# sloisel/MultiGridBarrier.jl

Hardware: AMD Instinct MI355X
Metric: Newton iters/sec + wall-clock to converge, 2D P2 p-Laplace L=9 (higher is better)
Workload: dtype f64

## Files before the change

include/mgbhip.h:

```cpp
#ifndef MGBHIP_H
#define MGBHIP_H

#include <stdint.h>

#ifdef __cplusplus
extern "C" {
#endif

#define MGBHIP_OK 0
#define MGBHIP_ERR_INVALID 1
#define MGBHIP_ERR_HIP 2
#define MGBHIP_ERR_NOT_SPD 3
#define MGBHIP_ERR_NONFINITE 4
#define MGBHIP_ERR_CONVERGENCE 5

#define MGBHIP_MAX_PIECES 4
#define MGBHIP_MAX_IDX 10
#define MGBHIP_MAX_LIN 4
#define MGBHIP_MAX_ND 13
#define MGBHIP_MAX_NU 4
#define MGBHIP_MAX_OPS 8

#define MGBHIP_KIND_EP 1
#define MGBHIP_KIND_LINEAR 2
// ... 139 lines not shown
                const mgbhip_vec* z0, mgbhip_vec* grad);
int mgbhip_f2_d(mgbhip_problem* prob, int32_t level, const mgbhip_vec* s, const mgbhip_vec* c,
                const mgbhip_vec* z0);
int mgbhip_solve_d(mgbhip_problem* prob, int32_t level, const mgbhip_vec* g, mgbhip_vec* x);
int mgbhip_prolong_add(mgbhip_problem* prob, int32_t level, const mgbhip_vec* s, mgbhip_vec* z);

int mgbhip_stage_ms(mgbhip_problem* prob, const char* stage, double* total_ms, int64_t* launches);
int mgbhip_reset_stage_timers(mgbhip_problem* prob, int enable);
int mgbhip_solver_stats(mgbhip_problem* prob, int32_t level, double* out8);
int mgbhip_solver_chain(mgbhip_problem* prob, int32_t level, double* out8);
enum { MGBHIP_PROJ_NONE = 0, MGBHIP_PROJ_LOOP = 1, MGBHIP_PROJ_STAGED = 2, MGBHIP_PROJ_MFMA = 3, MGBHIP_PROJ_ACCUMULATE = 4 };
int mgbhip_level_plan(mgbhip_problem* prob, int32_t level, int32_t* out16);
enum { MGBHIP_ELEM_F0 = 0, MGBHIP_ELEM_F1 = 1, MGBHIP_ELEM_F2 = 2, MGBHIP_ELEM_NODE_F = 3, MGBHIP_ELEM_NODE_SLACK = 4, MGBHIP_ELEM_F01 = 5 };
enum { MGBHIP_ELEM_KIND_DENSE = 0, MGBHIP_ELEM_KIND_WIDE = 1, MGBHIP_ELEM_KIND_FAST_DEFAULT = 2, MGBHIP_ELEM_KIND_FAST_RUNTIME = 3,
       MGBHIP_ELEM_KIND_CONDENSE = 4, MGBHIP_ELEM_KIND_GENERIC = 5 };
int mgbhip_elem_plan(mgbhip_problem* prob, int32_t mode, int32_t* out16);
int mgbhip_trial_values(mgbhip_problem* prob, int32_t level, const double* x, const double* dir, double step, const double* c,
                        const double* z0, double* y, double* g, double* xn, int32_t* moved, int32_t* finite, int32_t* path);
enum { MGBHIP_LAUNCH_ROW = 16 };
enum { MGBHIP_ASM_NONE = 0, MGBHIP_ASM_GATHER = 1, MGBHIP_ASM_COLUMNS = 2 };
enum { MGBHIP_B0_NA = 0, MGBHIP_B0_GATHER = 1, MGBHIP_B0_DIAG0 = 2, MGBHIP_B0_STEP0 = 3 };
enum { MGBHIP_BWD_NA = 0, MGBHIP_BWD_K8 = 1, MGBHIP_BWD_K16 = 2, MGBHIP_BWD_GENERAL = 3 };
int64_t mgbhip_solver_launches(mgbhip_problem* prob, int32_t level, int32_t* out, int64_t cap);

#define MGBHIP_INTERP_FEM1D 1
#define MGBHIP_INTERP_QK 2
#define MGBHIP_INTERP_P1 3
#define MGBHIP_INTERP_P2 4
#define MGBHIP_INTERP_SPECTRAL1D 5
#define MGBHIP_INTERP_SPECTRAL2D 6
#define MGBHIP_INTERP_P2C 7
int mgbhip_interpolate(mgbhip_ctx* ctx, int32_t family, int32_t d, int32_t k, int32_t p, int64_t N,
                       const double* x, const double* table, int32_t ncomp, const double* z, int64_t M,
                       const double* pts, double* out, int32_t* elem);
int mgbhip_interpolate_grad(mgbhip_ctx* ctx, int32_t family, int32_t d, int32_t k, int32_t p, int64_t N,
                            const double* x, const double* table, int32_t ncomp, const double* z, int64_t M,
                            const double* pts, double* out ,
                            double* grad , int32_t* elem );

typedef struct mgbhip_locator mgbhip_locator;
int mgbhip_locator_create(mgbhip_ctx* ctx, int32_t family, int32_t d, int32_t k, int32_t p, int64_t N,
                          const double* x, const double* table, int64_t M, const double* pts,
                          mgbhip_locator** out);
int mgbhip_locator_elements(const mgbhip_locator* loc, int32_t* elem );
int mgbhip_locator_evaluate(mgbhip_locator* loc, int32_t ncomp, const double* z ,
                            double* out ,
// ... 148 lines not shown
```

multigridbarrier.jl_amd/csrc/api.cpp:

```cpp
#include <chrono>
#include <cmath>
#include <cstring>
#include <algorithm>
#include <limits>
#include <memory>
#include <string>

#include "closest.hpp"
#include "contour.hpp"
#include "figure.hpp"
#include "interpolate.hpp"
#include "polyline.hpp"
#include "problem.hpp"
#include "quadrature.hpp"
#include "raycast.hpp"
#include "stream.hpp"
#include "surface.hpp"
#include "tubes.hpp"
#include "weld.hpp"

using namespace mgbhip;

mgbhip_problem* problem_create(mgbhip_ctx* ctx, const mgbhip_problem_desc* d, mgbhip_problem* share);
int core_run(mgbhip_problem* P, double* z, const double* c, const mgbhip_options* opt, mgbhip_core_result* res);
// ... 734 lines not shown
int mgbhip_solver_chain(mgbhip_problem* P, int32_t level, double* out) {
    MGB_API_BEGIN
    check_level(P, level);
    MGB_REQUIRE(out != nullptr, "null argument");
    MGB_REQUIRE(P->levels[level].solver.analyzed, "mgbhip_solver_chain: the level has not been factored yet");
    P->levels[level].solver.chain_stats(out);
    return MGBHIP_OK;
    MGB_API_END
}

static_assert(MGBHIP_LAUNCH_ROW == mgbhip::MF_LAUNCH_ROW && MGBHIP_ASM_GATHER == mgbhip::MF_ASM_GATHER &&
              MGBHIP_ASM_COLUMNS == mgbhip::MF_ASM_COLS && MGBHIP_B0_GATHER == mgbhip::MF_B0_GATHER &&
              MGBHIP_B0_DIAG0 == mgbhip::MF_B0_DIAG0 && MGBHIP_B0_STEP0 == mgbhip::MF_B0_STEP0 && MGBHIP_BWD_K8 == mgbhip::MF_BWD_K8 &&
              MGBHIP_BWD_K16 == mgbhip::MF_BWD_K16 && MGBHIP_BWD_GENERAL == mgbhip::MF_BWD_GENERAL, "mgbhip.h and mf_launch_plan.hpp disagree");

int64_t mgbhip_solver_launches(mgbhip_problem* P, int32_t level, int32_t* out, int64_t cap) {
    int64_t count = 0;
    const int rc = [&]() -> int {
        MGB_API_BEGIN
        check_level(P, level);
        MGB_REQUIRE(cap >= 0 && (out != nullptr || cap == 0), "bad output buffer");
        MGB_REQUIRE(P->levels[level].solver.analyzed, "mgbhip_solver_launches: the level has not been factored yet");
        count = P->levels[level].solver.launches(out, cap);
        return MGBHIP_OK;
        MGB_API_END
    }();
    return rc == MGBHIP_OK ? count : -(int64_t)rc;
}

#ifdef MGB_STEP_PROBE
int mgbhip_debug_probe(long long* out64) { (void)hipDeviceSynchronize(); mgbhip::mf_debug_probe(out64); return 0; }
#endif

int mgbhip_reset_stage_timers(mgbhip_problem* P, int enable) {
    MGB_API_BEGIN_ON(P)
    MGB_REQUIRE(P, "null argument");
    P->ctx->timers.reset(enable != 0);
    return MGBHIP_OK;
    MGB_API_END
}

static void interpolate_check_geometry(InterpIn& in) {
    const int32_t family = in.family, d = in.d, k = in.k, p = in.p;
    const int64_t N = in.N;
    const double* x = in.x;
    const bool fem = interp_is_fem(family);
// ... 799 lines not shown
```

multigridbarrier.jl_amd/csrc/mf_launch_plan.hpp:

```cpp
#pragma once
#include <algorithm>
#include <cstdint>
#include <cstdlib>
#include <vector>

#include "host_util.hpp"
#include "mf_analysis.hpp"

namespace mgbhip {

struct MfLaunch {
    int32_t first, count;
    int32_t cls;
    int32_t max_m, max_k;
    int32_t max_child = 0;
    bool tiny = false;
    bool wave = false;
    bool inv = false;
    bool iface = false;
    int32_t grec_first = -1;
};

constexpr int BIG_INV_MAX_M = 7000;
constexpr int GATHER_MAX_CHILD = 8;
constexpr int BIG_DIAG0_MIN_COUNT = 24;

struct MfSwitches {
    bool no_geo;
    bool old_big;
    bool merge_groups;
    bool packed_leaves;
    bool wave_small;
    int64_t inv_min_n;
    int64_t wave_min_n;
    bool gather_lds_maps;
    int gather_ct;
    bool bwd_split;
    static MfSwitches from_env() {
        auto num = [](const char* name, long long dflt) { const char* e = getenv(name); return e ? atoll(e) : dflt; };
        return {env_on("MGBHIP_NO_GEO"), env_on("MGBHIP_OLD_BIG"), !env_on("MGBHIP_NO_MERGE_GROUPS"), !env_on("MGBHIP_NO_PACKED_LEAVES"),
                !env_on("MGBHIP_NO_WAVE_SMALL"), num("MGBHIP_INV_MIN_N", 1024), num("MGBHIP_WAVE_MIN_N", 0),
                env_on("MGBHIP_GATHER_LDS_MAPS"), (int)num("MGBHIP_GATHER_CT", 0), num("MGBHIP_BWD_SPLIT", 1) != 0};
    }
};

using LevelLaunches = std::vector<std::vector<MfLaunch>>;

inline MfLaunch launch_of_range(const MfPlan& plan, MfLaunch L, int32_t first, int32_t count) {
    L.first = first; L.count = count;
    L.max_m = 0; L.max_k = 0; L.max_child = 0;
    for (int32_t t = first; t < first + count; ++t) {
        L.max_m = std::max(L.max_m, plan.fronts[t].m);
        L.max_k = std::max(L.max_k, plan.fronts[t].k);
        L.max_child = std::max(L.max_child, plan.fronts[t].nchild);
    }
    return L;
}

inline void merge_straggler_groups(const MfPlan& plan, std::vector<MfLaunch>& G) {
    auto absorb = [&](size_t into, size_t from) {
        MfLaunch& A = G[into];
        const MfLaunch& B = G[from];
        A.first = B.first;
        A.count += B.count;
        A.max_k = std::max(A.max_k, B.max_k);
// ... 143 lines not shown
    if (forced == 8 || forced == 16 || forced == 32) return forced;
    int ct = 8;
    while (ct < 32 && (int64_t)L.count * ((L.max_m + 2 * ct - 1) / (2 * ct)) >= GATHER_MIN_WGS) ct *= 2;
    return ct;
}

constexpr int BWD_SPLIT_MAX = 16;
constexpr int BWD_SPLIT_CUS = 256;
constexpr int BWD_SPLIT_COLS = 64;
constexpr int BWD_THIN_BOUNDARY = 8;
inline int bwd_inv_split(int32_t count, int32_t max_k, int32_t max_m) {
    if (count < 1 || max_m - max_k <= BWD_THIN_BOUNDARY) return 1;
    return std::max(1, std::min({BWD_SPLIT_MAX, BWD_SPLIT_CUS / count, (max_k + BWD_SPLIT_COLS - 1) / BWD_SPLIT_COLS}));
}
inline int32_t bwd_split_stride(int32_t max_k) { return (max_k + 1) & ~1; }
inline void bwd_split_scratch(const LevelLaunches& solves, int64_t out[2]) {
    out[0] = out[1] = 0;
    for (auto& lev : solves)
        for (auto& L : lev) {
            if (L.count == 0 || L.cls || !L.inv || bwd_inv_split(L.count, L.max_k, L.max_m) == 1) continue;
            out[0] = std::max<int64_t>(out[0], L.count);
            out[1] = std::max<int64_t>(out[1], (int64_t)L.count * bwd_split_stride(L.max_k));
        }
}

struct GatherRec {
    int64_t map_off;
    int64_t base[GATHER_MAX_CHILD];
    int32_t ld[GATHER_MAX_CHILD];
    int32_t bs[GATHER_MAX_CHILD];
};

inline void build_gather_maps(const MfPlan& plan, LevelLaunches& levels, std::vector<GatherRec>& recs, std::vector<int32_t>& gmap) {
    recs.clear();
    gmap.clear();
    for (auto& lev : levels)
        for (auto& L : lev) {
            L.grec_first = -1;
            if (L.count == 0 || big_assembly_kind(L) != MF_ASM_GATHER) continue;
            L.grec_first = (int32_t)recs.size();
            for (int32_t q = L.first; q < L.first + L.count; ++q) {
                const Front& f = plan.fronts[q];
                GatherRec R{};
                R.map_off = (int64_t)gmap.size();
                gmap.resize(gmap.size() + (size_t)f.nchild * (size_t)f.m, -1);
                for (int32_t c = 0; c < f.nchild; ++c) {
// ... 36 lines not shown
```

multigridbarrier.jl_amd/csrc/mf_numeric.hip:

```cpp
#include <hip/hip_runtime.h>

#include <cstdio>

#include <algorithm>
#include <cstdlib>

#include "../../include/mgbhip.h"
#include "mf_solver.hpp"
#include "mf_device.hpp"
#include "mf_small.hpp"
#include "mf_big_subst.hpp"
#include "mf_big_inv.hpp"

namespace mgbhip {

namespace {

int32_t query_lds_cap() {
    if (hipFuncSetAttribute((const void*)mf_factor_small<8, true>, hipFuncAttributeMaxDynamicSharedMemorySize,
                            (int)factor_small_lds(128)) == hipSuccess)
        return 128;
    (void)hipGetLastError();
    return 88;
}
// ... 137 lines not shown

    lds_cap = query_lds_cap();
    const bool inv_ok = !sw.old_big && query_inv_optin();
    level_launches = classify_launches(plan, lds_cap, inv_ok, sw);
    level_solves = merge_level_solves(level_launches);
    uses_inv = false;
    const std::vector<char> on_big_path = fronts_on_big_path(plan, level_launches);
    int32_t max_big = 1;
    for (auto& lev : level_launches)
        for (auto& L : lev) {
            uses_inv = uses_inv || L.inv;
            if (!L.cls) max_big = std::max(max_big, L.count);
        }
    d_dscr.alloc((size_t)max_big * 2 * NB * NB);
    {
        int64_t need[2] = {0, 0};
        if (sw.bwd_split) bwd_split_scratch(level_solves, need);
        if (need[0] == 0) { d_bwd_g.release(); d_bwd_cnt.release(); }
        else {
            d_bwd_g.alloc((size_t)need[1]);
            d_bwd_cnt.alloc((size_t)need[0]);
            d_bwd_cnt.zero(st);
        }
    }

    std::vector<int64_t> ug_ptr, ug_src;
    build_gather_lists(plan, on_big_path, fd, ug_ptr, ug_src);
    leaf_packed = sw.packed_leaves && pack_leaf_fronts(plan, level_launches, on_big_path, fd);
    d_ug_ptr.upload(ug_ptr, st);
    d_ug_src.upload(ug_src, st);
    std::vector<GatherRec> grec;
    std::vector<int32_t> gmap;
    if (!sw.gather_lds_maps) build_gather_maps(plan, level_launches, grec, gmap);
    gather_ct = sw.gather_ct;
    if (grec.empty()) { d_grec.release(); d_gmap.release(); }
    else { d_grec.upload(grec, st); d_gmap.upload(gmap, st); }
    d_fronts.upload(fd, st);
    h_fronts = fd;
    h_a_dst = remap_a_dst(plan, level_launches);
    d_a_dst.upload(h_a_dst, st);
    if (debug_level() >= 2) dump_plan(plan, level_launches);
    analyzed = true;
    MGB_HIP_CHECK(hipStreamSynchronize(st));
}

void MfSolver::set_direct_map(const int32_t* value_map, int64_t nnz, int64_t tail_base, hipStream_t st) {
// ... 86 lines not shown
    if (timers) timers->end();
}

void MfSolver::forward_pass(const double* d_b, hipStream_t st, StageTimers* timers) {
    y_border_one = false;
    y_zero = false;
    const SolveArgs a = solve_args(d_b, nullptr, st);
    int lvno = -1;
    for (auto& lev : level_solves) {
        LevelScope lvscope(timers, "fwd", ++lvno);
        for (auto& L : lev) {
            if (L.count == 0) continue;
            if (L.tiny) launch_forward_tiny(a, L);
            else if (L.cls) launch_forward_small(a, L);
            else if (L.inv && factored_inv) launch_fwd_inv(a, L);
            else if (L.max_m <= BIG1_MAX_M) launch_fwd_big1(a, L);
            else launch_fwd_big_steps(a, L);
        }
    }
}

void MfSolver::backward_pass(double* d_x, hipStream_t st, StageTimers* timers) {
    const SolveArgs a = solve_args(nullptr, d_x, st);
    for (int32_t l = (int32_t)level_solves.size() - 1; l >= 0; --l) {
        LevelScope lvscope(timers, "bwd", l);
        for (auto it = level_solves[l].rbegin(); it != level_solves[l].rend(); ++it) {
            const MfLaunch& L = *it;
            if (L.count == 0) continue;
            if (L.tiny) launch_backward_tiny(a, L);
            else if (L.cls) launch_backward_small(a, L);
            else if (L.inv && factored_inv) launch_bwd_inv(a, L);
            else if (L.max_m <= BIG1_MAX_M) launch_bwd_big1(a, L);
            else launch_bwd_big_steps(a, L);
        }
    }
}

#ifdef MGB_STEP_PROBE
void mf_debug_probe(long long* out64) {
    (void)hipMemcpyFromSymbol(out64, HIP_SYMBOL(g_probe), 64 * sizeof(long long));
    long long init[64];
    for (int i = 0; i < 64; ++i) init[i] = 0;
    init[56] = 0x7fffffffffffffffll;
    (void)hipMemcpyToSymbol(HIP_SYMBOL(g_probe), init, sizeof(init));
}
#endif

void MfSolver::chain_stats(double* out) const {
    double blocks = 0, big_levels = 0, fac = 0, bwd = 0, extra = 0;
    for (auto& lev : level_launches) {
        int lev_blocks = 0;
        for (auto& L : lev) {
            if (L.count == 0) continue;
            if (L.tiny || L.wave || L.cls) { fac += 1; continue; }
            const int nb = (L.max_k + NB - 1) / NB;
            lev_blocks = std::max(lev_blocks, nb);
            fac += 1 + nb + (L.iface ? 3 : 0);
            for (int32_t q = L.first; q < L.first + L.count; ++q) {
                const Front& f = plan.fronts[q];
                const double mk = (double)(f.m - f.k), steps = (double)((f.k + NB - 1) / NB);
                extra += 2.0 * 0.5 * (mk * mk + mk * f.k) * std::max(0.0, steps - 1.0);
            }
        }
        if (lev_blocks) { big_levels += 1; blocks += lev_blocks; }
    }
    for (auto& lev : level_solves)
        for (auto& L : lev)
            if (L.count) bwd += 1;
    out[0] = blocks; out[1] = big_levels; out[2] = fac; out[3] = bwd;
    out[4] = (double)plan.arena_doubles; out[5] = (double)plan.factor_flops; out[6] = extra; out[7] = 0.0;
}

int64_t MfSolver::launches(int32_t* out, int64_t cap) const {
    return launch_rows(level_launches, level_solves, leaf_packed, robust, out, cap);
}

void MfSolver::status_async(int32_t* h_dst2, hipStream_t st) const {
    MGB_HIP_CHECK(hipMemcpyAsync(h_dst2, d_status.p, 2 * sizeof(int32_t), hipMemcpyDeviceToHost, st));
}

int MfSolver::status(hipStream_t st) {
    int32_t h[2] = {0, 0};
    d_status.download(h, 2, st);
    MGB_HIP_CHECK(hipStreamSynchronize(st));
    return status_from(h, factored_condensed);
}

bool MfSolver::enable_condensed(int64_t N, int P, const int32_t* ucol, int64_t slack0, int64_t nnz, int64_t tail_base,
                                hipStream_t st) {
    condensed_ok = false;
    int why = 0;
// ... 70 lines not shown
```

multigridbarrier.jl_amd/csrc/mf_small.hpp:

```cpp
#pragma once
#include "mf_device.hpp"

namespace mgbhip {
namespace {

template <int NBT, bool PACKED>
__global__ void mf_factor_small(const FrontDev* __restrict__ fr, int32_t first,
                                const int32_t* __restrict__ children, const int32_t* __restrict__ rel,
                                const int32_t* __restrict__ a_src, const int32_t* __restrict__ a_dst,
                                const double* __restrict__ Hval, double* __restrict__ arena,
                                int32_t* __restrict__ status) {
    extern __shared__ double W[];
    const FrontDev F = fr[first + blockIdx.x];
    double* Fg = arena + F.F_off;
    const int m = F.m, k = F.k;
    const int tid = threadIdx.x, nt = blockDim.x;
    const int tx = tid % TX, ty = tid / TX, TYn = nt / TX;
    const int mm = PACKED ? m * (m + 1) / 2 : m * m;
    auto co = [m](int c) { return PACKED ? c * (m - 1) - c * (c - 1) / 2 : c * m; };
    double* S = W + mm;

    SP(0);
    int a_d0 = -1;
    double a_v0 = 0.0;
// ... 469 lines not shown
                if (two) s += l1[j] * t1;
                s = wave_sum_f64(s);
                if (lane == j) t0 -= s;
            }
        }
    } else {
        if (lane < m) t0 = (lane < k) ? y[idx[lane]] : x[idx[lane]];
        if (r1 < m) t1 = (r1 < k) ? y[idx[r1]] : x[idx[r1]];
#pragma unroll 2
        for (int j = k - 1; j >= 0; --j) {
            const double* Lj = Fm + (int64_t)j * m;
            double s = 0.0;
            if (lane > j && lane < m) s += Lj[lane] * t0;
            if (r1 > j && r1 < m) s += Lj[r1] * t1;
            s = wave_sum_f64(s);
            if (lane == j) t0 -= s;
            if (r1 == j) t1 -= s;
        }
    }
    if (lane < k) x[idx[lane]] = t0;
    if (r1 < k) x[idx[r1]] = t1;
}

__global__ __launch_bounds__(256) void mf_factor_tiny(const FrontDev* __restrict__ fr, int32_t first, int32_t count,
                                                      const int32_t* __restrict__ a_src,
                                                      const int32_t* __restrict__ a_dst,
                                                      const double* __restrict__ Hval, double* __restrict__ arena,
                                                      int32_t* __restrict__ status) {
    __shared__ double Wt[16][136];
    __shared__ double colb[16][16];
    const int g = threadIdx.x >> 4, r = threadIdx.x & 15;
    const int fi = blockIdx.x * 16 + g;
    const bool on = fi < count;
    const FrontDev F = fr[first + (on ? fi : 0)];
    const int m = F.m, k = on ? F.k : 0;
    double* W = Wt[g];
    for (int i = r; i < 136; i += 16) W[i] = 0.0;
    wave_sync();
    if (on)
        for (int t = r; t < F.a_cnt; t += 16) W[a_dst[F.a_off + t]] = Hval[a_src[F.a_off + t]];
    wave_sync();
    double a[16];
#pragma unroll
    for (int c = 0; c < 16; ++c) a[c] = (on && r < m && c <= r) ? W[c * 16 - c * (c - 1) / 2 + (r - c)] : 0.0;
    int kmax = k;
    kmax = max(kmax, __shfl_xor(kmax, 16, 64));
// ... 117 lines not shown
                       a.values, a.arena, a.status);
}

inline void launch_forward_tiny(const SolveArgs& a, const MfLaunch& L) {
    hipLaunchKernelGGL(mf_forward_tiny, dim3((L.count + 15) / 16), dim3(256), 0, a.st, a.fr, L.first, L.count, a.front_idx,
                       a.arena, a.b, a.y, a.uvec);
}
inline void launch_backward_tiny(const SolveArgs& a, const MfLaunch& L) {
    hipLaunchKernelGGL(mf_backward_tiny, dim3((L.count + 15) / 16), dim3(256), 0, a.st, a.fr, L.first, L.count, a.front_idx,
                       a.arena, a.y, a.x);
}

inline size_t forward_small_lds(int ts) { return (size_t)4 * ts * sizeof(double); }
inline void launch_forward_small(const SolveArgs& a, const MfLaunch& L) {
    const int ts = (L.max_m + 1) & ~1;
    hipLaunchKernelGGL(mf_forward_small, dim3((L.count + 3) / 4), dim3(256), forward_small_lds(ts), a.st, a.fr, L.first, L.count,
                       ts, a.front_idx, a.children, a.rel, a.arena, a.b, a.y, a.uvec);
}
template <int KMAX>
inline void launch_backward_small_k(const SolveArgs& a, const MfLaunch& L) {
    hipLaunchKernelGGL(mf_backward_small<KMAX>, dim3((L.count + 3) / 4), dim3(256), 0, a.st, a.fr, L.first, L.count, a.front_idx,
                       a.arena, a.y, a.x);
}
inline void launch_backward_small(const SolveArgs& a, const MfLaunch& L) {
    const int kmax = backward_small_kmax(L);
    if (kmax == 8) launch_backward_small_k<8>(a, L);
    else if (kmax == 16) launch_backward_small_k<16>(a, L);
    else launch_backward_small_k<0>(a, L);
}

}
}
```

multigridbarrier.jl_amd/csrc/mf_solver.hpp:

```cpp
#pragma once
#include <functional>

#include "common.hpp"
#include "mf_analysis.hpp"
#include "mf_launch_plan.hpp"
#include "kernels.hpp"

namespace mgbhip {

struct FrontDev {
    int32_t k, m, nchild, a_cnt;
    int64_t F_off, idx_off, u_off, child_off, rel_off, a_off, acol_off;
    int64_t ug_off;
    int32_t packed;
    int32_t pad_;
};

struct FactorArgs {
    const FrontDev* fr;
    const int32_t *children, *rel, *a_src, *a_dst, *a_colptr;
    const double* values;
    double *arena, *dscr, *dvec;
    int32_t* status;
    hipStream_t st;
    const GatherRec* grec;
    const int32_t* gmap;
    int gather_ct;
};
struct SolveArgs {
    const FrontDev* fr;
    const int32_t *front_idx, *children, *rel;
    const int64_t *ug_ptr, *ug_src;
    const double *arena, *dvec;
    const double* b;
    double *y, *x, *uvec, *tbig, *tsol;
    hipStream_t st;
    double* bwd_g;
    uint32_t* bwd_cnt;
};

class MfSolver {
   public:
    MfPlan plan;
    void analyze(int64_t n, const int32_t* rowptr, const int32_t* colidx, hipStream_t st,
                 const double* coords = nullptr, int dim = 0, bool protect_peeled = false,
                 const int32_t* top = nullptr, int64_t ntop = 0);
    std::function<void(double*, int64_t)> iface_reduce;
    void factor(const double* d_values, hipStream_t st, StageTimers* timers, bool direct = false, bool condensed = false);
    bool enable_condensed(int64_t N, int P, const int32_t* ucol, int64_t slack0, int64_t nnz, int64_t tail_base, hipStream_t st);
    bool condensed_ready() const { return condensed_ok; }
    bool leaves_packed() const { return leaf_packed; }
    const LeafDesc* leaf_desc() const { return d_leaf_desc.p; }
    double* arena() { return d_arena.p; }
    int32_t* leaf_status() { return d_status.p + 1; }
    const int32_t* status_flags() const { return d_status.p; }
    int32_t* status_flags_rw() { return d_status.p; }
    void flags_cleared() { status_zero = true; leaf_zero = true; }
    bool leaf_flag_zero() const { return leaf_zero; }
    void leaf_flag_used() { leaf_zero = false; }
    void set_direct_map(const int32_t* value_map, int64_t nnz, int64_t tail_base, hipStream_t st);
    bool has_direct_map() const { return d_a_src_direct.n > 0; }
    void solve(const double* d_b, double* d_x, hipStream_t st, StageTimers* timers);
    void solve_border(double* d_x_np1, hipStream_t st, StageTimers* timers);
    void chain_stats(double* out8) const;
    int64_t launches(int32_t* out, int64_t cap) const;
    int status(hipStream_t st);
    void status_async(int32_t* h_dst, hipStream_t st) const;
    static int status_from(const int32_t* flags2, bool with_leaves) {
        return (flags2[0] || (with_leaves && flags2[1])) ? MGBHIP_ERR_NOT_SPD : MGBHIP_OK;
    }
    bool factored_condensed = false;
    bool analyzed = false;
    bool robust = false;
    bool has_inverse_path() const { return uses_inv; }
    bool factored_inv = false;

   private:
    void upload_plan(hipStream_t st);
    SolveArgs solve_args(const double* d_b, double* d_x, hipStream_t st) const {
        return {d_fronts.p, d_front_idx.p, d_children.p, d_rel.p, d_ug_ptr.p, d_ug_src.p, d_arena.p, d_dvec.p, d_b, d_y.p, d_x,
                d_uvec.p, d_tbig.p, d_tsol.p, st, d_bwd_g.p, d_bwd_cnt.n ? d_bwd_cnt.p : nullptr};
    }
    void forward_pass(const double* d_b_np1, hipStream_t st, StageTimers* timers);
    void backward_pass(double* d_x_np1, hipStream_t st, StageTimers* timers);
    DevBuf<double> d_bx, d_xx, d_one;
    DevBuf<FrontDev> d_fronts;
    DevBuf<int32_t> d_front_idx, d_children, d_rel, d_a_src, d_a_src_direct, d_a_dst, d_a_colptr;
    DevBuf<GatherRec> d_grec;
    DevBuf<int32_t> d_gmap;
    DevBuf<int64_t> d_ug_ptr, d_ug_src;
    DevBuf<double> d_arena, d_uvec, d_y, d_tbig, d_tsol, d_dscr, d_dvec;
    DevBuf<double> d_ifpack;
    DevBuf<int32_t> d_status;
    DevBuf<double> d_bwd_g;
    DevBuf<uint32_t> d_bwd_cnt;
    bool condensed_ok = false;
    bool leaf_packed = false;
    std::vector<FrontDev> h_fronts;
    std::vector<int32_t> h_a_dst;
    DevBuf<FrontDev> d_fronts_c;
    DevBuf<int32_t> d_a_src_c, d_a_dst_c, d_a_colptr_c;
    DevBuf<LeafDesc> d_leaf_desc;
    std::vector<std::vector<MfLaunch>> level_launches;
    std::vector<std::vector<MfLaunch>> level_solves;
    int gather_ct = 0;
    int32_t lds_cap = 88;
    bool uses_inv = false;
    bool y_border_one = false;
    bool y_zero = false;
    bool status_zero = false, leaf_zero = false;
};

}
```

multigridbarrier.jl_amd/device.py:

```python
from __future__ import annotations

import ctypes as C
import os
import weakref
from typing import List, Optional

import numpy as np
import scipy.sparse as sp

from .blockmatrices import BlockColumn, BlockDiag
from .convex import KIND_EP, KIND_LINEAR, Convex
from .multigrid import AMG
from .problem import MGBProblem

MAX_PIECES, MAX_IDX, MAX_ND, MAX_NU, MAX_OPS = 4, 10, 13, 4, 8
MAX_LIN = 4
OK, ERR_INVALID, ERR_HIP, ERR_NOT_SPD, ERR_NONFINITE, ERR_CONVERGENCE = range(6)


class Device:
    """reference: src/device.jl:18"""


class CPUDevice(Device):
# ... 55 lines not shown
EARLY_FN = C.CFUNCTYPE(C.c_int, C.POINTER(C.c_double), C.c_double, C.c_void_p)
ALLREDUCE_FN = C.CFUNCTYPE(C.c_int, C.c_void_p, C.c_void_p, C.c_int64, C.c_int32, C.c_int32)


class _CoreResult(C.Structure):
    _fields_ = [("k", C.c_int32), ("L", C.c_int32), ("failure_code", C.c_int32), ("t_final", C.c_double),
                ("t_elapsed", C.c_double), ("solve_seconds", C.c_double), ("newton_iterations", C.c_int64),
                ("f0_evals", C.c_int64), ("f1_evals", C.c_int64), ("f2_evals", C.c_int64),
                ("factorizations", C.c_int64), ("cap_steps", C.c_int32), ("its", C.POINTER(C.c_int64)),
                ("ts", _dp), ("kappas", _dp), ("times", _dp), ("c_dot_Dz", _dp)]


EXPORTS = [
    "mgbhip_create", "mgbhip_destroy", "mgbhip_last_error", "mgbhip_version", "mgbhip_problem_create",
    "mgbhip_problem_destroy", "mgbhip_problem_set_box", "mgbhip_problem_set_barrier_weights",
    "mgbhip_level_size", "mgbhip_f0", "mgbhip_f1", "mgbhip_f2", "mgbhip_hessian_pattern", "mgbhip_solve",
    "mgbhip_set_hessian", "mgbhip_solve_newton", "mgbhip_newton_direction", "mgbhip_problem_set_sharding",
    "mgbhip_problem_set_collective",
    "mgbhip_node_barrier", "mgbhip_node_slack", "mgbhip_mgb_core", "mgbhip_matched_t",
    "mgbhip_default_options", "mgbhip_stage_ms", "mgbhip_reset_stage_timers", "mgbhip_solver_stats", "mgbhip_solver_chain",
    "mgbhip_vec_alloc", "mgbhip_vec_free", "mgbhip_vec_len", "mgbhip_vec_upload", "mgbhip_vec_download",
    "mgbhip_vec_fill", "mgbhip_vec_copy", "mgbhip_vec_axpy", "mgbhip_vec_scale", "mgbhip_vec_dot",
    "mgbhip_vec_norm", "mgbhip_vec_isfinite", "mgbhip_f0_d", "mgbhip_f1_d", "mgbhip_f2_d", "mgbhip_solve_d",
    "mgbhip_prolong_add", "mgbhip_level_plan", "mgbhip_elem_plan", "mgbhip_trial_values", "mgbhip_solver_launches", "mgbhip_interpolate", "mgbhip_interpolate_grad",
    "mgbhip_locator_create", "mgbhip_locator_elements", "mgbhip_locator_evaluate", "mgbhip_locator_destroy",
    "mgbhip_closest_create", "mgbhip_closest_fetch", "mgbhip_closest_evaluate", "mgbhip_closest_destroy",
    "mgbhip_quadrature_create", "mgbhip_quadrature_points", "mgbhip_quadrature_weights", "mgbhip_quadrature_integrate",
    "mgbhip_quadrature_max", "mgbhip_quadrature_plan", "mgbhip_quadrature_times", "mgbhip_quadrature_destroy",
    "mgbhip_contour_create", "mgbhip_contour_fetch", "mgbhip_contour_destroy", "mgbhip_contour_create_embedded",
    "mgbhip_tessellate_create", "mgbhip_tessellate_fetch", "mgbhip_tessellate_destroy",
    "mgbhip_weld_create", "mgbhip_weld_fetch", "mgbhip_weld_rounds", "mgbhip_weld_destroy",
    "mgbhip_polyline_create", "mgbhip_polyline_fetch", "mgbhip_polyline_rounds", "mgbhip_polyline_destroy",
    "mgbhip_polyline_sample",
    "mgbhip_raycast_create", "mgbhip_raycast_offsets", "mgbhip_raycast_samples", "mgbhip_raycast_lengths",
    "mgbhip_raycast_integrate", "mgbhip_raycast_render", "mgbhip_raycast_destroy", "mgbhip_raycast_render_layers",
    "mgbhip_surface_create", "mgbhip_surface_trace", "mgbhip_surface_shade", "mgbhip_surface_destroy",
    "mgbhip_stream_create", "mgbhip_stream_set_field", "mgbhip_stream_trace", "mgbhip_stream_destroy",
    "mgbhip_tubes_create", "mgbhip_tubes_trace", "mgbhip_tubes_shade", "mgbhip_tubes_destroy",
    "mgbhip_figure_create", "mgbhip_figure_render", "mgbhip_figure_render_rgba8", "mgbhip_figure_counts",
    "mgbhip_figure_destroy",
]


def library_path() -> str:
    here = os.path.dirname(os.path.abspath(__file__))
    return os.environ.get("MGBHIP_LIB") or os.path.join(here, "lib", "libmgbhip.so")

# ... 24 lines not shown
        getattr(lib, name).argtypes = [C.c_void_p, C.c_int32, _dp, _dp, _dp, _dp]
    lib.mgbhip_hessian_pattern.argtypes = [C.c_void_p, C.c_int32, C.POINTER(C.c_int64), C.POINTER(_ip), C.POINTER(_ip)]
    lib.mgbhip_solve.argtypes = [C.c_void_p, C.c_int32, _dp, _dp]
    lib.mgbhip_set_hessian.argtypes = [C.c_void_p, C.c_int32, _dp]
    lib.mgbhip_solve_newton.argtypes = [C.c_void_p, C.c_int32, _dp, _dp, _dp]
    lib.mgbhip_newton_direction.argtypes = [C.c_void_p, C.c_int32, _dp, _dp, _dp, _dp, _dp, _ip]
    lib.mgbhip_problem_set_sharding.argtypes = [C.c_void_p, C.c_int32, C.c_int64, _ip, _dp]
    lib.mgbhip_problem_set_collective.argtypes = [C.c_void_p, C.c_void_p, C.c_void_p, C.c_int32]
    lib.mgbhip_node_barrier.argtypes = [C.c_void_p, _dp, _dp, _dp]
    lib.mgbhip_node_slack.argtypes = [C.c_void_p, _dp, _dp]
    lib.mgbhip_mgb_core.argtypes = [C.c_void_p, _dp, _dp, C.POINTER(Options), C.POINTER(_CoreResult)]
    lib.mgbhip_matched_t.argtypes = [C.c_void_p, _dp, _dp, C.c_double, _dp]
    lib.mgbhip_default_options.argtypes = [C.POINTER(Options), C.c_int64]
    lib.mgbhip_default_options.restype = None
    lib.mgbhip_stage_ms.argtypes = [C.c_void_p, C.c_char_p, _dp, C.POINTER(C.c_int64)]
    lib.mgbhip_reset_stage_timers.argtypes = [C.c_void_p, C.c_int]
    lib.mgbhip_solver_stats.argtypes = [C.c_void_p, C.c_int32, _dp]
    lib.mgbhip_solver_chain.argtypes = [C.c_void_p, C.c_int32, _dp]
    lib.mgbhip_level_plan.argtypes = [C.c_void_p, C.c_int32, _ip]
    lib.mgbhip_elem_plan.argtypes = [C.c_void_p, C.c_int32, _ip]
    lib.mgbhip_trial_values.argtypes = [C.c_void_p, C.c_int32, _dp, _dp, C.c_double, _dp, _dp, _dp, _dp, _dp, _ip, _ip, _ip]
    lib.mgbhip_solver_launches.argtypes = [C.c_void_p, C.c_int32, _ip, C.c_int64]
    lib.mgbhip_solver_launches.restype = C.c_int64
    vp = C.c_void_p
    lib.mgbhip_vec_alloc.argtypes = [vp, C.c_int64, C.POINTER(vp)]
    lib.mgbhip_vec_free.argtypes = [vp]
    lib.mgbhip_vec_len.argtypes = [vp]
    lib.mgbhip_vec_len.restype = C.c_int64
    lib.mgbhip_vec_upload.argtypes = [vp, _dp, C.c_int64]
    lib.mgbhip_vec_download.argtypes = [vp, _dp, C.c_int64]
    lib.mgbhip_vec_fill.argtypes = [vp, C.c_double]
    lib.mgbhip_vec_copy.argtypes = [vp, vp]
    lib.mgbhip_vec_axpy.argtypes = [C.c_double, vp, vp]
    lib.mgbhip_vec_scale.argtypes = [C.c_double, vp]
    lib.mgbhip_vec_dot.argtypes = [vp, vp, _dp]
    lib.mgbhip_vec_norm.argtypes = [vp, _dp]
    lib.mgbhip_vec_isfinite.argtypes = [vp, C.POINTER(C.c_int32)]
    lib.mgbhip_f0_d.argtypes = [vp, C.c_int32, vp, vp, vp, _dp]
    lib.mgbhip_f1_d.argtypes = [vp, C.c_int32, vp, vp, vp, vp]
    lib.mgbhip_f2_d.argtypes = [vp, C.c_int32, vp, vp, vp]
    lib.mgbhip_solve_d.argtypes = [vp, C.c_int32, vp, vp]
    lib.mgbhip_prolong_add.argtypes = [vp, C.c_int32, vp, vp]
    lib.mgbhip_interpolate.argtypes = [vp, C.c_int32, C.c_int32, C.c_int32, C.c_int32, C.c_int64, _dp, _dp, C.c_int32,
                                       _dp, C.c_int64, _dp, _dp, _ip]
    lib.mgbhip_interpolate_grad.argtypes = [vp, C.c_int32, C.c_int32, C.c_int32, C.c_int32, C.c_int64, _dp, _dp,
                                            C.c_int32, _dp, C.c_int64, _dp, _dp, _dp, _ip]
# ... 523 lines not shown
    BACKWARD = ("n/a", "k8", "k16", "general")

    @classmethod
    def launch_rows(cls, raw) -> list:
        rows = []
        for r in np.asarray(raw, dtype=np.int64).reshape(-1, 16):
            d = dict(zip(cls.LAUNCH_KEYS, (int(v) for v in r)))
            for k in ("tiny", "wave", "inv", "iface", "packed"):
                d[k] = bool(d[k])
            d["assembly"], d["block0"], d["backward"] = cls.ASSEMBLY[d["assembly"]], cls.BLOCK0[d["block0"]], cls.BACKWARD[d["backward"]]
            rows.append(d)
        return rows

    def solver_launches(self, level: int) -> list:
        n = self.lib.mgbhip_solver_launches(self.handle, level, None, 0)
        if n < 0:
            _check(self.lib, int(-n))
        out = (C.c_int32 * (16 * max(int(n), 1)))()
        n = self.lib.mgbhip_solver_launches(self.handle, level, out, n)
        if n < 0:
            _check(self.lib, int(-n))
        return self.launch_rows(np.frombuffer(out, dtype=np.int32)[:16 * int(n)])

    def close(self):
        if self.handle:
            self.lib.mgbhip_problem_destroy(self.handle)
            self.handle = None

    def __del__(self):
        try:
            self.close()
        except Exception:
            pass


def dense_as_block(M: AMG) -> AMG:
    if isinstance(M.D_fine[0], BlockColumn):
        return M
    n = M.w.size
    geom = M.geometry
    ops = {k: BlockDiag(np.asarray(v, dtype=np.float64).reshape(n, n, 1)) for k, v in geom.operators.items()}
    from dataclasses import replace
    g2 = replace(geom, operators=ops)
    nu = len(M.state_names)
    D_fine = [BlockColumn(ops[name], state, nu) for (state, name) in M.D_spec]
    return AMG(geometry=g2, x=M.x, w=M.w, R_fine=M.R_fine, D_fine=D_fine, state_names=M.state_names, D_spec=M.D_spec)
# ... 47 lines not shown
```

Before: 693.5.

## Fuse consecutive backward-solve tree levels into per-subtree kernels

Groups consecutive elimination-tree levels of the multifrontal backward solve into subtrees. Each subtree is processed by one workgroup that walks the levels top-down with __syncthreads between them, so one kernel launch replaces one launch per level. This targets launch and serialization overhead in the many small backward solves per Newton step. The cost is less parallelism per launch, since grid size equals the subtree root count, plus uneven work per block and extra plan data uploaded to the device.

```diff
diff --git a/include/mgbhip.h b/include/mgbhip.h
--- a/include/mgbhip.h
+++ b/include/mgbhip.h
@@ -185,6 +185,8 @@
 enum { MGBHIP_B0_NA = 0, MGBHIP_B0_GATHER = 1, MGBHIP_B0_DIAG0 = 2, MGBHIP_B0_STEP0 = 3 };
 enum { MGBHIP_BWD_NA = 0, MGBHIP_BWD_K8 = 1, MGBHIP_BWD_K16 = 2, MGBHIP_BWD_GENERAL = 3 };
 int64_t mgbhip_solver_launches(mgbhip_problem* prob, int32_t level, int32_t* out, int64_t cap);
+enum { MGBHIP_BWD_GROUP_ROW = 6 };
+int64_t mgbhip_solver_bwd_groups(mgbhip_problem* prob, int32_t level, int32_t* out, int64_t cap);
 
 #define MGBHIP_INTERP_FEM1D 1
 #define MGBHIP_INTERP_QK 2
diff --git a/multigridbarrier.jl_amd/csrc/api.cpp b/multigridbarrier.jl_amd/csrc/api.cpp
--- a/multigridbarrier.jl_amd/csrc/api.cpp
+++ b/multigridbarrier.jl_amd/csrc/api.cpp
@@ -780,6 +780,22 @@
         MGB_REQUIRE(cap >= 0 && (out != nullptr || cap == 0), "bad output buffer");
         MGB_REQUIRE(P->levels[level].solver.analyzed, "mgbhip_solver_launches: the level has not been factored yet");
         count = P->levels[level].solver.launches(out, cap);
+        return MGBHIP_OK;
+        MGB_API_END
+    }();
+    return rc == MGBHIP_OK ? count : -(int64_t)rc;
+}
+
+static_assert(MGBHIP_BWD_GROUP_ROW == mgbhip::MF_BWD_GROUP_ROW, "mgbhip.h and mf_launch_plan.hpp disagree");
+
+int64_t mgbhip_solver_bwd_groups(mgbhip_problem* P, int32_t level, int32_t* out, int64_t cap) {
+    int64_t count = 0;
+    const int rc = [&]() -> int {
+        MGB_API_BEGIN
+        check_level(P, level);
+        MGB_REQUIRE(cap >= 0 && (out != nullptr || cap == 0), "bad output buffer");
+        MGB_REQUIRE(P->levels[level].solver.analyzed, "mgbhip_solver_bwd_groups: the level has not been factored yet");
+        count = P->levels[level].solver.bwd_group_report(out, cap);
         return MGBHIP_OK;
         MGB_API_END
     }();
diff --git a/multigridbarrier.jl_amd/csrc/mf_launch_plan.hpp b/multigridbarrier.jl_amd/csrc/mf_launch_plan.hpp
--- a/multigridbarrier.jl_amd/csrc/mf_launch_plan.hpp
+++ b/multigridbarrier.jl_amd/csrc/mf_launch_plan.hpp
@@ -36,11 +36,13 @@
     bool gather_lds_maps;
     int gather_ct;
     bool bwd_split;
+    bool bwd_fuse;
     static MfSwitches from_env() {
         auto num = [](const char* name, long long dflt) { const char* e = getenv(name); return e ? atoll(e) : dflt; };
         return {env_on("MGBHIP_NO_GEO"), env_on("MGBHIP_OLD_BIG"), !env_on("MGBHIP_NO_MERGE_GROUPS"), !env_on("MGBHIP_NO_PACKED_LEAVES"),
                 !env_on("MGBHIP_NO_WAVE_SMALL"), num("MGBHIP_INV_MIN_N", 1024), num("MGBHIP_WAVE_MIN_N", 0),
-                env_on("MGBHIP_GATHER_LDS_MAPS"), (int)num("MGBHIP_GATHER_CT", 0), num("MGBHIP_BWD_SPLIT", 1) != 0};
+                env_on("MGBHIP_GATHER_LDS_MAPS"), (int)num("MGBHIP_GATHER_CT", 0), num("MGBHIP_BWD_SPLIT", 1) != 0,
+                num("MGBHIP_BWD_FUSE", 1) != 0};
     }
 };
 
@@ -230,6 +232,122 @@
             out[0] = std::max<int64_t>(out[0], L.count);
             out[1] = std::max<int64_t>(out[1], (int64_t)L.count * bwd_split_stride(L.max_k));
         }
+}
+
+constexpr int BWD_FUSE_R = 2;
+constexpr int BWD_FUSE_MIN_ROOTS = 32;
+struct BwdGroup {
+    int32_t top = 0, bottom = 0;
+    int32_t roots = 0;
+    int32_t fronts = 0;
+    int32_t max_seg = 0;
+    int64_t seg_off = 0;
+    int32_t nseg() const { return top - bottom + 1; }
+    bool fused() const { return top > bottom; }
+};
+inline bool bwd_level_fusable(const std::vector<MfLaunch>& solves) {
+    int live = 0;
+    for (auto& L : solves) {
+        if (L.count == 0) continue;
+        if (!L.cls || L.tiny) return false;
+        ++live;
+    }
+    return live == 1;
+}
+inline std::vector<BwdGroup> fuse_backward_levels(const MfPlan& plan, const LevelLaunches& solves, const MfSwitches& sw) {
+    std::vector<BwdGroup> groups;
+    const int32_t nlev = (int32_t)solves.size();
+    auto width = [&](int32_t l) { return plan.level_ptr[l + 1] - plan.level_ptr[l]; };
+    for (int32_t l = nlev - 1; l >= 0;) {
+        if (!bwd_level_fusable(solves[l])) { --l; continue; }
+        BwdGroup G;
+        G.top = G.bottom = l;
+        G.roots = G.fronts = width(l);
+        const bool enough_roots = width(l) == 1 || width(l) >= BWD_FUSE_MIN_ROOTS;
+        while (sw.bwd_fuse && enough_roots && G.bottom > 0 && bwd_level_fusable(solves[G.bottom - 1]) &&
+               (int64_t)width(G.bottom - 1) <= (int64_t)4 * BWD_FUSE_R * G.roots) {
+            --G.bottom;
+            G.fronts += width(G.bottom);
+            for (int32_t q = plan.level_ptr[G.bottom]; q < plan.level_ptr[G.bottom + 1]; ++q) {
+                const int32_t par = plan.fronts[q].parent;
+                if (par < 0 || plan.fronts[par].level > G.top) ++G.roots;
+            }
+        }
+        groups.push_back(G);
+        l = G.bottom - 1;
+    }
+    return groups;
+}
+
+struct BwdItem {
+    int32_t front, kmax;
+    int32_t k, m;
+    int64_t F_off, idx_off;
+};
+struct BwdSubtreeLists {
+    std::vector<int32_t> seg_ptr;
+    std::vector<BwdItem> items;
+};
+inline void build_backward_subtrees(const MfPlan& plan, const LevelLaunches& solves, std::vector<BwdGroup>& groups, BwdSubtreeLists& out) {
+    out.seg_ptr.clear();
+    out.items.clear();
+    std::vector<int32_t> root_of(plan.fronts.size(), -1);
+    for (auto& G : groups) {
+        G.max_seg = 1;
+        G.seg_off = 0;
+        if (!G.fused()) continue;
+        const int32_t S = G.nseg();
+        int32_t nroots = 0;
+        for (int32_t l = G.top; l >= G.bottom; --l)
+            for (int32_t q = plan.level_ptr[l]; q < plan.level_ptr[l + 1]; ++q) {
+                const int32_t par = plan.fronts[q].parent;
+                root_of[q] = (par < 0 || plan.fronts[par].level > G.top) ? nroots++ : root_of[par];
+            }
+        G.seg_off = (int64_t)out.seg_ptr.size();
+        const size_t base = out.seg_ptr.size();
+        out.seg_ptr.resize(base + (size_t)nroots * S + 1, 0);
+        int32_t* ptr = out.seg_ptr.data() + base;
+        for (int32_t l = G.top; l >= G.bottom; --l)
+            for (int32_t q = plan.level_ptr[l]; q < plan.level_ptr[l + 1]; ++q) ++ptr[(int64_t)root_of[q] * S + (G.top - l) + 1];
+        const int32_t item0 = (int32_t)out.items.size();
+        ptr[0] = item0;
+        for (int64_t i = 1; i <= (int64_t)nroots * S; ++i) {
+            G.max_seg = std::max(G.max_seg, ptr[i]);
+            ptr[i] += ptr[i - 1];
+        }
+        out.items.resize((size_t)ptr[(int64_t)nroots * S]);
+        std::vector<int32_t> fill(ptr, ptr + (int64_t)nroots * S);
+        for (int32_t l = G.top; l >= G.bottom; --l) {
+            int32_t kmax = 0;
+            for (auto& L : solves[l])
+                if (L.count) kmax = backward_small_kmax(L);
+            for (int32_t q = plan.level_ptr[l]; q < plan.level_ptr[l + 1]; ++q)
+                out.items[(size_t)fill[(int64_t)root_of[q] * S + (G.top - l)]++] =
+                    BwdItem{q, kmax, plan.fronts[q].k, plan.fronts[q].m, plan.fronts[q].F_off, plan.fronts[q].idx_off};
+        }
+    }
+}
+
+inline int64_t backward_launch_count(const LevelLaunches& solves, const std::vector<BwdGroup>& groups) {
+    int64_t n = 0;
+    for (auto& lev : solves)
+        for (auto& L : lev)
+            if (L.count) ++n;
+    for (auto& G : groups)
+        if (G.fused()) n -= G.nseg() - 1;
+    return n;
+}
+constexpr int MF_BWD_GROUP_ROW = 6;
+inline int64_t bwd_group_rows(const std::vector<BwdGroup>& groups, int32_t* out, int64_t cap) {
+    int64_t n = 0;
+    for (auto& G : groups) {
+        if (n < cap && out) {
+            int32_t* r = out + n * MF_BWD_GROUP_ROW;
+            r[0] = G.top; r[1] = G.bottom; r[2] = G.roots; r[3] = G.fronts; r[4] = G.max_seg; r[5] = G.fused();
+        }
+        ++n;
+    }
+    return n;
 }
 
 struct GatherRec {
diff --git a/multigridbarrier.jl_amd/csrc/mf_numeric.hip b/multigridbarrier.jl_amd/csrc/mf_numeric.hip
--- a/multigridbarrier.jl_amd/csrc/mf_numeric.hip
+++ b/multigridbarrier.jl_amd/csrc/mf_numeric.hip
@@ -183,6 +183,14 @@
             d_bwd_cnt.alloc((size_t)need[0]);
             d_bwd_cnt.zero(st);
         }
+    }
+
+    {
+        bwd_groups = fuse_backward_levels(plan, level_solves, sw);
+        BwdSubtreeLists lists;
+        build_backward_subtrees(plan, level_solves, bwd_groups, lists);
+        if (lists.items.empty()) { d_bwd_seg.release(); d_bwd_items.release(); }
+        else { d_bwd_seg.upload(lists.seg_ptr, st); d_bwd_items.upload(lists.items, st); }
     }
 
     std::vector<int64_t> ug_ptr, ug_src;
@@ -315,7 +323,15 @@
 
 void MfSolver::backward_pass(double* d_x, hipStream_t st, StageTimers* timers) {
     const SolveArgs a = solve_args(nullptr, d_x, st);
+    size_t g = 0;
     for (int32_t l = (int32_t)level_solves.size() - 1; l >= 0; --l) {
+        while (g < bwd_groups.size() && (!bwd_groups[g].fused() || bwd_groups[g].top > l)) ++g;
+        if (g < bwd_groups.size() && bwd_groups[g].top == l) {
+            LevelScope lvscope(timers, "bwd", l);
+            launch_backward_subtree(a, bwd_groups[g]);
+            l = bwd_groups[g].bottom;
+            continue;
+        }
         LevelScope lvscope(timers, "bwd", l);
         for (auto it = level_solves[l].rbegin(); it != level_solves[l].rend(); ++it) {
             const MfLaunch& L = *it;
@@ -357,9 +373,7 @@
         }
         if (lev_blocks) { big_levels += 1; blocks += lev_blocks; }
     }
-    for (auto& lev : level_solves)
-        for (auto& L : lev)
-            if (L.count) bwd += 1;
+    bwd = (double)backward_launch_count(level_solves, bwd_groups);
     out[0] = blocks; out[1] = big_levels; out[2] = fac; out[3] = bwd;
     out[4] = (double)plan.arena_doubles; out[5] = (double)plan.factor_flops; out[6] = extra; out[7] = 0.0;
 }
diff --git a/multigridbarrier.jl_amd/csrc/mf_small.hpp b/multigridbarrier.jl_amd/csrc/mf_small.hpp
--- a/multigridbarrier.jl_amd/csrc/mf_small.hpp
+++ b/multigridbarrier.jl_amd/csrc/mf_small.hpp
@@ -515,6 +515,77 @@
     if (r1 < k) x[idx[r1]] = t1;
 }
 
+template <int KMAX>
+__device__ __forceinline__ void backward_small_front(const BwdItem& F, int lane, const int32_t* front_idx, const double* arena,
+                                                     const double* y, double* x) {
+    const int m = F.m, k = F.k;
+    const int32_t* idx = front_idx + F.idx_off;
+    const double* Fm = arena + F.F_off;
+    const int r1 = lane + 64;
+    double t0 = 0.0, t1 = 0.0;
+    if constexpr (KMAX > 0) {
+        double l0[KMAX], l1[KMAX];
+        const bool two = m > 64;
+#pragma unroll
+        for (int j = 0; j < KMAX; ++j) {
+            l0[j] = (j < k && lane > j && lane < m) ? Fm[(int64_t)j * m + lane] : 0.0;
+            l1[j] = (two && j < k && r1 < m) ? Fm[(int64_t)j * m + r1] : 0.0;
+        }
+        if (lane < m) t0 = (lane < k) ? y[idx[lane]] : x[idx[lane]];
+        if (r1 < m) t1 = (r1 < k) ? y[idx[r1]] : x[idx[r1]];
+#pragma unroll
+        for (int j = KMAX - 1; j >= 0; --j) {
+            if (j < k) {
+                double s = l0[j] * t0;
+                if (two) s += l1[j] * t1;
+                s = wave_sum_f64(s);
+                if (lane == j) t0 -= s;
+            }
+        }
+    } else {
+        if (lane < m) t0 = (lane < k) ? y[idx[lane]] : x[idx[lane]];
+        if (r1 < m) t1 = (r1 < k) ? y[idx[r1]] : x[idx[r1]];
+#pragma unroll 2
+        for (int j = k - 1; j >= 0; --j) {
+            const double* Lj = Fm + (int64_t)j * m;
+            double s = 0.0;
+            if (lane > j && lane < m) s += Lj[lane] * t0;
+            if (r1 > j && r1 < m) s += Lj[r1] * t1;
+            s = wave_sum_f64(s);
+            if (lane == j) t0 -= s;
+            if (r1 == j) t1 -= s;
+        }
+    }
+    if (lane < k) x[idx[lane]] = t0;
+    if (r1 < k) x[idx[r1]] = t1;
+}
+
+__global__ __launch_bounds__(256) void mf_backward_subtree(const int32_t* __restrict__ seg_ptr, const BwdItem* __restrict__ items,
+                                                           int32_t nseg, const int32_t* __restrict__ front_idx,
+                                                           const double* __restrict__ arena, const double* y, double* x) {
+    const int lane = threadIdx.x & 63, wave = threadIdx.x >> 6;
+    const int32_t* sp = seg_ptr + (int64_t)blockIdx.x * nseg;
+    int begin = sp[0], end = sp[1];
+    BwdItem first{};
+    if (begin + wave < end) first = items[begin + wave];
+    for (int s = 0; s < nseg; ++s) {
+        const int next_end = (s + 1 < nseg) ? sp[s + 2] : end;
+        BwdItem next_first{};
+        if (s + 1 < nseg && end + wave < next_end) next_first = items[end + wave];
+        for (int i = begin + wave; i < end; i += 4) {
+            const BwdItem it = (i == begin + wave) ? first : items[i];
+            const int kmax = __builtin_amdgcn_readfirstlane(it.kmax);
+            if (kmax == 8) backward_small_front<8>(it, lane, front_idx, arena, y, x);
+            else if (kmax == 16) backward_small_front<16>(it, lane, front_idx, arena, y, x);
+            else backward_small_front<0>(it, lane, front_idx, arena, y, x);
+        }
+        __syncthreads();
+        begin = end;
+        end = next_end;
+        first = next_first;
+    }
+}
+
 __global__ __launch_bounds__(256) void mf_factor_tiny(const FrontDev* __restrict__ fr, int32_t first, int32_t count,
                                                       const int32_t* __restrict__ a_src,
                                                       const int32_t* __restrict__ a_dst,
@@ -678,6 +749,10 @@
     hipLaunchKernelGGL(mf_backward_small<KMAX>, dim3((L.count + 3) / 4), dim3(256), 0, a.st, a.fr, L.first, L.count, a.front_idx,
                        a.arena, a.y, a.x);
 }
+inline void launch_backward_subtree(const SolveArgs& a, const BwdGroup& G) {
+    hipLaunchKernelGGL(mf_backward_subtree, dim3(G.roots), dim3(256), 0, a.st, a.bwd_seg + G.seg_off, a.bwd_items, G.nseg(),
+                       a.front_idx, a.arena, a.y, a.x);
+}
 inline void launch_backward_small(const SolveArgs& a, const MfLaunch& L) {
     const int kmax = backward_small_kmax(L);
     if (kmax == 8) launch_backward_small_k<8>(a, L);
diff --git a/multigridbarrier.jl_amd/csrc/mf_solver.hpp b/multigridbarrier.jl_amd/csrc/mf_solver.hpp
--- a/multigridbarrier.jl_amd/csrc/mf_solver.hpp
+++ b/multigridbarrier.jl_amd/csrc/mf_solver.hpp
@@ -37,6 +37,8 @@
     hipStream_t st;
     double* bwd_g;
     uint32_t* bwd_cnt;
+    const int32_t* bwd_seg;
+    const BwdItem* bwd_items;
 };
 
 class MfSolver {
@@ -62,6 +64,7 @@
     bool has_direct_map() const { return d_a_src_direct.n > 0; }
     void solve(const double* d_b, double* d_x, hipStream_t st, StageTimers* timers);
     void solve_border(double* d_x_np1, hipStream_t st, StageTimers* timers);
+    int64_t bwd_group_report(int32_t* out, int64_t cap) const { return bwd_group_rows(bwd_groups, out, cap); }
     void chain_stats(double* out8) const;
     int64_t launches(int32_t* out, int64_t cap) const;
     int status(hipStream_t st);
@@ -79,7 +82,7 @@
     void upload_plan(hipStream_t st);
     SolveArgs solve_args(const double* d_b, double* d_x, hipStream_t st) const {
         return {d_fronts.p, d_front_idx.p, d_children.p, d_rel.p, d_ug_ptr.p, d_ug_src.p, d_arena.p, d_dvec.p, d_b, d_y.p, d_x,
-                d_uvec.p, d_tbig.p, d_tsol.p, st, d_bwd_g.p, d_bwd_cnt.n ? d_bwd_cnt.p : nullptr};
+                d_uvec.p, d_tbig.p, d_tsol.p, st, d_bwd_g.p, d_bwd_cnt.n ? d_bwd_cnt.p : nullptr, d_bwd_seg.p, d_bwd_items.p};
     }
     void forward_pass(const double* d_b_np1, hipStream_t st, StageTimers* timers);
     void backward_pass(double* d_x_np1, hipStream_t st, StageTimers* timers);
@@ -94,6 +97,9 @@
     DevBuf<int32_t> d_status;
     DevBuf<double> d_bwd_g;
     DevBuf<uint32_t> d_bwd_cnt;
+    std::vector<BwdGroup> bwd_groups;
+    DevBuf<int32_t> d_bwd_seg;
+    DevBuf<BwdItem> d_bwd_items;
     bool condensed_ok = false;
     bool leaf_packed = false;
     std::vector<FrontDev> h_fronts;
diff --git a/multigridbarrier.jl_amd/device.py b/multigridbarrier.jl_amd/device.py
--- a/multigridbarrier.jl_amd/device.py
+++ b/multigridbarrier.jl_amd/device.py
@@ -101,7 +101,7 @@
     "mgbhip_vec_alloc", "mgbhip_vec_free", "mgbhip_vec_len", "mgbhip_vec_upload", "mgbhip_vec_download",
     "mgbhip_vec_fill", "mgbhip_vec_copy", "mgbhip_vec_axpy", "mgbhip_vec_scale", "mgbhip_vec_dot",
     "mgbhip_vec_norm", "mgbhip_vec_isfinite", "mgbhip_f0_d", "mgbhip_f1_d", "mgbhip_f2_d", "mgbhip_solve_d",
-    "mgbhip_prolong_add", "mgbhip_level_plan", "mgbhip_elem_plan", "mgbhip_trial_values", "mgbhip_solver_launches", "mgbhip_interpolate", "mgbhip_interpolate_grad",
+    "mgbhip_prolong_add", "mgbhip_level_plan", "mgbhip_elem_plan", "mgbhip_trial_values", "mgbhip_solver_launches", "mgbhip_solver_bwd_groups", "mgbhip_interpolate", "mgbhip_interpolate_grad",
     "mgbhip_locator_create", "mgbhip_locator_elements", "mgbhip_locator_evaluate", "mgbhip_locator_destroy",
     "mgbhip_closest_create", "mgbhip_closest_fetch", "mgbhip_closest_evaluate", "mgbhip_closest_destroy",
     "mgbhip_quadrature_create", "mgbhip_quadrature_points", "mgbhip_quadrature_weights", "mgbhip_quadrature_integrate",
@@ -172,6 +172,9 @@
     lib.mgbhip_trial_values.argtypes = [C.c_void_p, C.c_int32, _dp, _dp, C.c_double, _dp, _dp, _dp, _dp, _dp, _ip, _ip, _ip]
     lib.mgbhip_solver_launches.argtypes = [C.c_void_p, C.c_int32, _ip, C.c_int64]
     lib.mgbhip_solver_launches.restype = C.c_int64
+    if hasattr(lib, "mgbhip_solver_bwd_groups"):
+        lib.mgbhip_solver_bwd_groups.argtypes = [C.c_void_p, C.c_int32, _ip, C.c_int64]
+        lib.mgbhip_solver_bwd_groups.restype = C.c_int64
     vp = C.c_void_p
     lib.mgbhip_vec_alloc.argtypes = [vp, C.c_int64, C.POINTER(vp)]
     lib.mgbhip_vec_free.argtypes = [vp]
@@ -741,6 +744,19 @@
             _check(self.lib, int(-n))
         return self.launch_rows(np.frombuffer(out, dtype=np.int32)[:16 * int(n)])
 
+    BWD_GROUP_KEYS = ("top", "bottom", "roots", "fronts", "max_seg", "fused")
+
+    def solver_bwd_groups(self, level: int) -> list:
+        n = self.lib.mgbhip_solver_bwd_groups(self.handle, level, None, 0)
+        if n < 0:
+            _check(self.lib, int(-n))
+        out = (C.c_int32 * (6 * max(int(n), 1)))()
+        n = self.lib.mgbhip_solver_bwd_groups(self.handle, level, out, n)
+        if n < 0:
+            _check(self.lib, int(-n))
+        rows = np.frombuffer(out, dtype=np.int32)[:6 * int(n)].reshape(-1, 6)
+        return [dict(zip(self.BWD_GROUP_KEYS, (int(v) for v in r))) for r in rows]
+
     def close(self):
         if self.handle:
             self.lib.mgbhip_problem_destroy(self.handle)
```

After: 692.8 (median of 2 runs). No clear change (-0.1%).
